# struan-robertson/shoeprint-image-retrieval

Measured on AMD Instinct MI355X. Metric: query x gallery NCC pairs/sec, higher is better.
Workload: dtype f32; 1 GPU; config 2: WVU2019-shaped VGG16 conv3_3 NCC: Q=100 x G=1500 (1500/GPU), features [256,128,64] stored as float32, rotations/scales none, queries signal 1 / noise 126; method=fft, gallery_chunk=1500, storage=float32, parallelism=gallery-shard x1, streams=1

## Files before the change

shoeprint-image-retrieval_amd/csrc/ncc_fft.hip:

```cpp
#include <cstdlib>

#include "fft_core.h"
#include "ncc_fft_cfg.h"
#include "ncc_prep_common.h"

#ifndef SPR_BIG_ABL
#define SPR_BIG_ABL 0
#endif
namespace spr {
namespace {

inline int rt_stride(int r_rows) { return r_rows + ((8 - r_rows % 32) + 32) % 32; }

template <class C, bool BIG, int PT>
__global__ void __launch_bounds__(PT)
prep_fft_kernel(NccGeom g, int is_query, const void* __restrict__ maps, unsigned char* __restrict__ prepared,
                size_t item_bytes, const cf* __restrict__ tw_h, const cf* __restrict__ tw_w, unsigned x0_off,
                unsigned f_off, unsigned xbuf_off, unsigned zbuf_off, unsigned sat2_off, int f_stride,
                unsigned char* __restrict__ ws, size_t slot_bytes) {
  using GH = typename C::GH;
  using GW = typename C::GW;
  unsigned char* lds = dyn_lds();
  unsigned char* big = lds;
  if constexpr (BIG) big = ws + (static_cast<size_t>(blockIdx.y) * gridDim.x + blockIdx.x) * slot_bytes;
// ... 516 lines not shown
#pragma unroll
          for (int s = 0; s < KW; ++s) {
            const cf v = y[pp][s];
            const int e = (pp * KW + s) * 2;
            const int n2 = GW::out_index(tr, pp, s);
            const int n1 = 2 * (rr * C::PPR + gr);
            const bool ok = GW::out_valid(tr, pp) && n2 < g.iw;
            if (ok && n1 < g.ih) maps_out[(static_cast<size_t>(c) * g.ih + n1) * g.iw + n2] = v.x * ivf[e];
            if (ok && n1 + 1 < g.ih) maps_out[(static_cast<size_t>(c) * g.ih + n1 + 1) * g.iw + n2] = v.y * ivf[e + 1];
          }
        }
      }
    }
    store_nyq();
    __syncthreads();
  }

  float best = 0.0f;
#pragma unroll
  for (int r = 0; r < RR; ++r)
#pragma unroll
    for (int e = 0; e < NV; ++e) best = fmaxf(best, acc[r][e]);
  best = block_max<C::NT>(best, red);
  if (tid == 0 && scores) {
    const float s = best / static_cast<float>(g.channels);
    float* dst = scores + static_cast<size_t>(qi) * ld + col0 + gi_item;
    const float prev = g.accumulate ? *dst : 0.0f;
    *dst = s > prev ? s : prev;
  }
  }
}

struct PrepFftLds {
  size_t x0_off, f_off, xbuf_off, zbuf_off, sat2_off, total;
  int f_stride;
  size_t slot_bytes;
};
template <class C>
PrepFftLds prep_fft_lds(const NccGeom& g, bool is_query, int pt) {
  const int h = is_query ? g.th : g.ih, w = is_query ? g.tw : g.iw;
  PrepFftLds l;
  l.f_stride = C::NW / 2 + 1;
  const size_t f_bytes = sizeof(cf) * static_cast<size_t>(2 * ((h + 1) / 2)) * l.f_stride;
  const size_t sat_bytes = align_up(sizeof(double) * (h + 1) * (w + 1), 16);
  if (g.big) {
    l.xbuf_off = 64;
    l.zbuf_off = l.xbuf_off;
    l.total = l.xbuf_off + sizeof(cf) * C::prep_xbuf_elems(pt);
    l.x0_off = 0;
    l.f_off = align_up(sizeof(float) * h * w, 256);
    const size_t first = f_bytes > sat_bytes ? f_bytes : sat_bytes;
    l.sat2_off = align_up(l.f_off + first, 256);
    l.slot_bytes = align_up(l.sat2_off + (is_query ? 0 : sat_bytes), 256);
    return l;
  }
  l.slot_bytes = 0;
  l.x0_off = 64;
  l.f_off = align_up(l.x0_off + sizeof(float) * h * w, 16);
  l.xbuf_off = align_up(l.f_off + f_bytes, 16);
  l.zbuf_off = l.xbuf_off;
  const size_t fft_total = l.xbuf_off + sizeof(cf) * C::prep_xbuf_elems(pt);
  size_t sat_total = is_query ? 0 : l.f_off + sat_bytes;
  l.sat2_off = 0;
  if (!is_query && l.f_off + 2 * sat_bytes <= static_cast<size_t>(kLdsLimit)) {
    l.sat2_off = l.f_off + sat_bytes;
    sat_total = l.f_off + 2 * sat_bytes;
  }
  l.total = fft_total > sat_total ? fft_total : sat_total;
  return l;
}

struct PairFftLds {
  size_t r_off, xbuf_off, nyq_off, total, slot_bytes;
};
template <class C>
constexpr int rk_tuned() { return C::RR_A * C::PPR * 2 < C::NH ? C::RR_A * C::PPR * 2 : C::NH; }

template <class C>
PairFftLds pair_fft_lds(const NccGeom& g) {
  PairFftLds l;
  l.r_off = 64;
  const size_t r_bytes = sizeof(cf) * static_cast<size_t>(C::COLS) * g.r_stride;
  l.slot_bytes = g.big ? align_up(r_bytes, 256) : 0;
  l.xbuf_off = align_up(l.r_off + (g.big ? 0 : r_bytes), 16);
  l.nyq_off = align_up(l.xbuf_off + sizeof(cf) * C::xbuf_elems(C::NT), 16);
  l.total = l.nyq_off + sizeof(cf) * (2 * C::NH + C::NH + C::NW);
  return l;
}

struct FftEntry {
  int nh, nw, eh, tgh, ew, tgw, nt, spl_w;
  int kw_a, rr_a, kw_b, rr_b, rk_a;
  bool pow2;
  int spec_per_chan;
  size_t (*prep_lds_total)(const NccGeom&, bool);
  size_t (*pair_lds_total)(const NccGeom&);
  int (*prep)(const NccGeom&, const PlanScratch&, const PrepCall&);
  int (*pair)(const NccGeom&, const PlanScratch&, const PairCall&);
  size_t (*prep_slot_bytes)(const NccGeom&, bool);
  size_t (*pair_slot_bytes)(const NccGeom&);
  bool big_only;
  bool six;
};

template <class C>
int prep_threads(const NccGeom& g, bool q) {
  if (C::NH * C::NW >= 128 * 64 && prep_fft_lds<C>(g, q, 512).total <= static_cast<size_t>(kLdsLimit)) return 512;
  return kThreads;
}
template <class C>
size_t prep_lds_total_t(const NccGeom& g, bool q) { return prep_fft_lds<C>(g, q, prep_threads<C>(g, q)).total; }
template <class C>
size_t pair_lds_total_t(const NccGeom& g) { return pair_fft_lds<C>(g).total; }
template <class C>
size_t prep_slot_bytes_t(const NccGeom& g, bool q) { return prep_fft_lds<C>(g, q, kThreads).slot_bytes; }
template <class C>
size_t pair_slot_bytes_t(const NccGeom& g) { return pair_fft_lds<C>(g).slot_bytes; }

template <class C, bool BIG, int PT>
int prep_launch(const NccGeom& g, const PlanScratch& s, const PrepCall& c) {
  const PrepFftLds l = prep_fft_lds<C>(g, c.is_query, PT);
  const size_t item_bytes = c.is_query ? prepared_query_item_bytes(g, SPR_NCC_FFT) : prepared_gallery_item_bytes(g, SPR_NCC_FFT);
  (void)hipFuncSetAttribute(reinterpret_cast<const void*>(prep_fft_kernel<C, BIG, PT>),
                            hipFuncAttributeMaxDynamicSharedMemorySize, kLdsLimit);
  int64_t batch = c.n;
  if (BIG) {
    const size_t per_item = l.slot_bytes * static_cast<size_t>(g.channels);
    if (!s.ws || s.ws_bytes < per_item) { set_error("prep_fft_kernel: workspace too small for one item"); return SPR_ERR_WORKSPACE; }
    batch = static_cast<int64_t>(s.ws_bytes / per_item);
  }
  const int raw_h = c.is_query ? g.q_h : g.g_h, raw_w = c.is_query ? g.q_w : g.g_w;
  const size_t elem = g.dtype == SPR_F32 ? 4 : 2;
  const size_t raw_item_bytes = static_cast<size_t>(g.channels) * raw_h * raw_w * elem;
  for (int64_t first = 0; first < c.n; first += batch) {
    const int64_t m = c.n - first < batch ? c.n - first : batch;
    hipLaunchKernelGGL(HIP_KERNEL_NAME(prep_fft_kernel<C, BIG, PT>), dim3(g.channels, static_cast<unsigned>(m)), dim3(PT),
                       l.total, c.stream, g, c.is_query ? 1 : 0,
                       static_cast<const void*>(static_cast<const unsigned char*>(c.maps) + first * raw_item_bytes),
                       static_cast<unsigned char*>(c.prepared) + first * item_bytes, item_bytes, s.tw_h,
                       s.tw_w, static_cast<unsigned>(l.x0_off), static_cast<unsigned>(l.f_off),
                       static_cast<unsigned>(l.xbuf_off), static_cast<unsigned>(l.zbuf_off),
                       static_cast<unsigned>(l.sat2_off), l.f_stride, static_cast<unsigned char*>(s.ws), l.slot_bytes);
    const int rc = check_launch("prep_fft_kernel");
    if (rc != SPR_OK) return rc;
  }
  return SPR_OK;
}
template <class C>
int prep_t(const NccGeom& g, const PlanScratch& s, const PrepCall& c) {
#ifndef SPR_SAN_SUBSET
  if (g.big) return prep_launch<C, true, kThreads>(g, s, c);
#endif
  if (prep_threads<C>(g, c.is_query) == 512) return prep_launch<C, false, 512>(g, s, c);
  return prep_launch<C, false, kThreads>(g, s, c);
}

constexpr int kTeamCounters = 8 * 32;

template <class C, int RR, int KW, int PF, int RK, bool BIG, bool TEAM>
int pair_launch(const NccGeom& g, const PlanScratch& s, const PairCall& c) {
  const int64_t nq = c.nq, ng = c.ng;
  unsigned* team_sync = c.maps_out && !BIG ? nullptr : s.team_sync;
  const PairFftLds l = pair_fft_lds<C>(g);
  const int64_t tiles = static_cast<int64_t>(ceil_div(static_cast<int>(nq), kTileQ)) * ceil_div(static_cast<int>(ng), kTileG);
  PairArgs a{};
  a.channels = g.channels; a.nq = static_cast<int>(nq); a.ng = static_cast<int>(ng);
  a.ih = g.ih; a.iw = g.iw; a.r_rows = g.r_rows; a.r_stride = g.r_stride; a.rounds_r = g.rounds_r;
  a.inv_per_chan = g.inv_per_chan; a.accumulate = c.accumulate;
  const void* kernel = reinterpret_cast<const void*>(pair_fft_kernel<C, RR, KW, PF, RK, BIG, TEAM>);
  (void)hipFuncSetAttribute(kernel, hipFuncAttributeMaxDynamicSharedMemorySize, kLdsLimit);
  unsigned grid = 0;
  int per_cu = 0, cus = 0, dev = 0;
  if (TEAM && !team_sync) { set_error("pair_fft_kernel: the team schedule needs the plan's counters"); return SPR_ERR_ARG; }
  if (TEAM && hipGetDevice(&dev) == hipSuccess &&
      hipDeviceGetAttribute(&cus, hipDeviceAttributeMultiprocessorCount, dev) == hipSuccess &&
      hipOccupancyMaxActiveBlocksPerMultiprocessor(&per_cu, pair_fft_kernel<C, RR, KW, PF, RK, BIG, TEAM>, C::NT, l.total) == hipSuccess &&
      per_cu > 0 && cus >= 8) {
    int team_size = cus / 8 * per_cu;
    if (BIG) {
      const size_t slots = s.ws ? s.ws_bytes / l.slot_bytes : 0;
      if (slots < 8) { set_error("pair_fft_kernel: workspace too small"); return SPR_ERR_WORKSPACE; }
      if (static_cast<size_t>(team_size) * 8 > slots) team_size = static_cast<int>(slots / 8);
    }
    {
      const int strip_max = env_int("SPR_NCC_STRIP_Q", 16) > 0 ? env_int("SPR_NCC_STRIP_Q", 16) : 16;
      const int strips = ceil_div(static_cast<int>(nq), strip_max);
      a.team_size = team_size;
      a.strips = strips;
      a.strip_q = ceil_div(static_cast<int>(nq), strips);
      a.strips = ceil_div(static_cast<int>(nq), a.strip_q);
      a.epochs_full = static_cast<int>((static_cast<int64_t>(a.strip_q) * ng + team_size - 1) / team_size);
      const int q_last = static_cast<int>(nq) - (a.strips - 1) * a.strip_q;
      a.epochs_total = (a.strips - 1) * a.epochs_full + static_cast<int>((static_cast<int64_t>(q_last) * ng + team_size - 1) / team_size);
      a.sync_polls = env_int("SPR_NCC_TEAM_POLLS", BIG ? 0 : 256);
      a.sync_every = env_int("SPR_NCC_TEAM_EVERY", BIG ? 0 : 32);
      if (a.sync_every < 0) a.sync_every = 0;
      grid = 8u * static_cast<unsigned>(team_size);
      if (hipMemsetAsync(team_sync, 0, sizeof(unsigned) * kTeamCounters, c.stream) != hipSuccess) {
        set_error("hipMemsetAsync(team counters) failed");
        return SPR_ERR_HIP;
      }
    }
  }
  if (TEAM && a.team_size == 0) { set_error("pair_fft_kernel: could not size the persistent grid"); return SPR_ERR_HIP; }
  const int64_t max_tiles = TEAM ? tiles : pair_tiles_per_launch(kTileQ * kTileG, C::NT);
  for (int64_t t0 = 0; t0 < (TEAM ? 1 : tiles); t0 += max_tiles) {
    if (!TEAM) {
      const int64_t n = tiles - t0 < max_tiles ? tiles - t0 : max_tiles;
      a.tile0 = static_cast<int>(t0);
      grid = static_cast<unsigned>(n * kTileQ * kTileG);
    }
    hipLaunchKernelGGL(HIP_KERNEL_NAME(pair_fft_kernel<C, RR, KW, PF, RK, BIG, TEAM>), dim3(grid),
                       dim3(C::NT), l.total, c.stream, a, static_cast<const unsigned char*>(c.pq),
                       prepared_query_item_bytes(g, SPR_NCC_FFT), static_cast<const unsigned char*>(c.pg),
                       prepared_gallery_item_bytes(g, SPR_NCC_FFT), c.scores,
                       static_cast<long long>(c.ld), static_cast<long long>(c.col0), c.maps_out, s.tw_h, s.tw_w,
                       static_cast<unsigned>(l.r_off), static_cast<unsigned>(l.xbuf_off),
                       static_cast<unsigned>(l.nyq_off), team_sync, static_cast<unsigned char*>(s.ws), l.slot_bytes);
    const int rc = check_launch("pair_fft_kernel");
    if (rc != SPR_OK) return rc;
  }
  (void)kernel;
  return SPR_OK;
}

constexpr int kBigMidKw = 11, kBigMidRr = 4;
template <class C, int PFA, bool BIG, bool TEAM>
int pair_tb(const NccGeom& g, const PlanScratch& s, const PairCall& c) {
  if (g.tight) return pair_launch<C, C::RR_A, C::KW_A, PFA, rk_tuned<C>(), BIG, TEAM>(g, s, c);
  if constexpr (BIG) {
    if (g.keep_w == kBigMidKw) return pair_launch<C, kBigMidRr, kBigMidKw, 1, 0, BIG, TEAM>(g, s, c);
  }
  return pair_launch<C, C::RR_B, C::KW_B, 1, 0, BIG, TEAM>(g, s, c);
}
template <class C, int PFA>
int pair_t(const NccGeom& g, const PlanScratch& s, const PairCall& c) {
#ifndef SPR_SAN_SUBSET
  if (g.big) return pair_tb<C, PFA, true, true>(g, s, c);
  if (s.team_sync && !c.maps_out && team_schedule()) return pair_tb<C, PFA, false, true>(g, s, c);
#endif
  return pair_tb<C, PFA, false, false>(g, s, c);
}

template <class C, int PFA, bool BIG_ONLY = false>
constexpr FftEntry entry() {
  return FftEntry{C::NH,   C::NW,   C::EH,   C::TGH,  C::EW,   C::TGW, C::NT, C::GW::SPL,
                  C::KW_A, C::RR_A, C::KW_B, C::RR_B, rk_tuned<C>(),
                  (C::NH & (C::NH - 1)) == 0 && (C::NW & (C::NW - 1)) == 0,
                  C::kSpecPerChan, prep_lds_total_t<C>, pair_lds_total_t<C>, prep_t<C>, pair_t<C, PFA>,
                  prep_slot_bytes_t<C>, pair_slot_bytes_t<C>, BIG_ONLY, false};
}

size_t pair6_lds_total(const NccGeom&) { return pair6_lds_bytes(); }
size_t no_slot_bytes(const NccGeom&) { return 0; }
template <class C>
constexpr FftEntry entry6() {
  return FftEntry{C::NH, C::NW, C::EH, C::TGH, C::EW, C::TGW, C::NT, C::GW::SPL, 0, 0, 0, 0, 0, false,
                  C::kSpecPerChan, prep_lds_total_t<C>, pair6_lds_total, prep_t<C>, launch_pair6,
                  prep_slot_bytes_t<C>, no_slot_bytes, false, true};
}

#ifdef SPR_SAN_SUBSET
const FftEntry kEntries[] = {
    entry<Cfg<8, 4, 4, 4, 64, 2, 1>, 1>(),
    entry<Cfg<12, 8, 6, 8, 192, 5, 2>, 1>(),
    entry6<Cfg<12, 16, 12, 8, 384, 5, 2, 1>>(),
    entry<Cfg<12, 16, 12, 8, 256, 5, 2>, 1>(),
};
#else
const FftEntry kEntries[] = {
    entry<Cfg<8, 4, 4, 4, 64, 2, 1>, 1>(),
    entry<Cfg<8, 4, 8, 4, 64, 2, 1>, 1>(),
    entry<Cfg<12, 4, 6, 4, 64, 2, 1>, 1>(),
    entry<Cfg<8, 8, 8, 4, 64, 2, 1>, 1>(),
    entry<Cfg<8, 8, 8, 8, 256, 4, 1>, 1>(),
    entry<Cfg<12, 8, 6, 8, 192, 5, 2>, 1>(),
    entry<Cfg<16, 8, 8, 8, 256, 4, 1>, 1>(),
    entry<Cfg<16, 8, 16, 8, 256, 4, 1>, 1>(),
    entry6<Cfg<12, 16, 12, 8, 384, 5, 2, 1>>(),
    entry<Cfg<12, 16, 12, 8, 256, 5, 2>, 1>(),
    entry<Cfg<16, 16, 16, 8, 512, 4, 1>, 2>(),
    entry<Cfg<24, 16, 12, 16, 512, 9, 4>, 1, true>(),
};
#endif

const FftEntry* find_entry(int nh, int nw, int six) {
  for (const FftEntry& e : kEntries)
    if (e.nh == nh && e.nw == nw && (e.six ? 1 : 0) == six) return &e;
  return nullptr;
}

inline int fft_need(int img, int tpl) {
  const int c = tpl / 2;
  const int a = img + c, b = img + tpl - 1 - c;
  return a > b ? a : b;
}

bool fill_geometry(NccGeom& g, const FftEntry& e, bool big) {
  g.big = big ? 1 : 0;
  g.six = e.six ? 1 : 0;
  g.nh = e.nh; g.nw = e.nw; g.eh = e.eh; g.tgh = e.tgh; g.ew = e.ew; g.tgw = e.tgw; g.nt = e.nt;
  if (e.six) {
    if (big || env_int("SPR_NCC_SIX", 1) == 0) return false;
    if (g.ih > pair6_max_rows() || g.iw > pair6_max_cols()) return false;
    g.rounds_c = 2; g.r_rows = g.ih; g.r_stride = 0; g.rounds_r = 1; g.tight = 1; g.keep_w = 0; g.nv = 24;
    g.spec_per_chan = e.spec_per_chan;
    g.inv_per_chan = 6 * e.nt * 4;
    if (g.ih * g.iw > kMaxPixPerThread * kThreads || g.th * g.tw > kMaxPixPerThread * kThreads) return false;
    if (e.prep_lds_total(g, true) > static_cast<size_t>(kLdsLimit)) return false;
    if (e.prep_lds_total(g, false) > static_cast<size_t>(kLdsLimit)) return false;
    return e.pair_lds_total(g) <= static_cast<size_t>(kLdsLimit);
  }
  const int cpr = e.nt / e.tgh, ppr = e.nt / e.tgw;
  g.rounds_c = ceil_div(e.nw / 2, cpr);
  g.r_rows = (g.ih + 7) / 8 * 8;
  if (g.r_rows > e.nh) g.r_rows = e.nh;
  g.rounds_r = ceil_div(g.r_rows / 2, ppr);
  const int kw_need = ceil_div(g.iw, e.ew);
  const bool tuned = kw_need <= e.kw_a && g.rounds_r <= e.rr_a;
  g.r_stride = rt_stride(tuned ? e.rk_a : g.r_rows);
  g.tight = tuned ? 1 : 0;
  g.keep_w = tuned ? e.kw_a : e.kw_b;
  if (!tuned && (kw_need > e.kw_b || g.rounds_r > e.rr_b)) return false;
  if (big && !tuned && kw_need <= kBigMidKw && g.rounds_r <= kBigMidRr && kBigMidKw < e.kw_b) g.keep_w = kBigMidKw;
  g.nv = (e.spl_w * g.keep_w * 2 + 3) / 4 * 4;
  g.spec_per_chan = e.spec_per_chan;
  g.inv_per_chan = g.rounds_r * g.nv * e.nt;
  if (!big && (g.ih * g.iw > kMaxPixPerThread * kThreads || g.th * g.tw > kMaxPixPerThread * kThreads)) return false;
  if (e.prep_lds_total(g, true) > static_cast<size_t>(kLdsLimit)) return false;
  if (e.prep_lds_total(g, false) > static_cast<size_t>(kLdsLimit)) return false;
  if (e.pair_lds_total(g) > static_cast<size_t>(kLdsLimit)) return false;
  return true;
}

}

bool fft_geometry(NccGeom& g, bool pow2_only) {
  const int need_h = fft_need(g.ih, g.th), need_w = fft_need(g.iw, g.tw);
  const int min_h = need_h > g.th ? need_h : g.th, min_w = need_w > g.tw ? need_w : g.tw;
  const FftEntry* best = nullptr;
  NccGeom best_g = g;
  const bool force_big = env_int("SPR_NCC_FORCE_BIG", 0) == 1;
#ifdef SPR_SAN_SUBSET
  constexpr int kPasses = 1;
#else
  constexpr int kPasses = 2;
#endif
  for (int pass = force_big ? 1 : 0; pass < kPasses && !best; ++pass) {
    for (const FftEntry& e : kEntries) {
      if (e.nh < min_h || e.nw < min_w) continue;
      if (pow2_only && !e.pow2) continue;
      if (pass == 0 && e.big_only) continue;
      if (best && static_cast<long long>(e.nh) * e.nw >= static_cast<long long>(best->nh) * best->nw) continue;
      NccGeom trial = g;
      if (!fill_geometry(trial, e, pass == 1)) continue;
      best = &e;
      best_g = trial;
    }
  }
  if (!best) return false;
  g = best_g;
  return true;
}

size_t fft_workspace_bytes(const NccGeom& g) {
  if (!g.big) return 0;
  const FftEntry* e = find_entry(g.nh, g.nw, g.six);
  if (!e) return 0;
  const size_t prep_q = e->prep_slot_bytes(g, true), prep_g = e->prep_slot_bytes(g, false);
  const size_t prep = (prep_q > prep_g ? prep_q : prep_g) * static_cast<size_t>(g.channels) * 2;
  const size_t pair = e->pair_slot_bytes(g) * 512;
  return prep > pair ? prep : pair;
}

int launch_prep_fft(const NccGeom& g, const PlanScratch& s, const PrepCall& c) {
  if (c.n == 0) return SPR_OK;
  const FftEntry* e = find_entry(g.nh, g.nw, g.six);
  if (!e) { set_error("no FFT kernel for grid %dx%d", g.nh, g.nw); return SPR_ERR_UNSUPPORTED; }
  return e->prep(g, s, c);
}

int launch_pair_fft(const NccGeom& g, const PlanScratch& s, const PairCall& c) {
  if (c.nq == 0 || c.ng == 0) return SPR_OK;
  const FftEntry* e = find_entry(g.nh, g.nw, g.six);
  if (!e) { set_error("no FFT kernel for grid %dx%d", g.nh, g.nw); return SPR_ERR_UNSUPPORTED; }
  return e->pair(g, s, c);
}

#ifdef SPR_PREP_STAMPS
extern "C" int spr_debug_read_prep_stamps(unsigned long long* host, int n) {
  return hipMemcpyFromSymbol(host, HIP_SYMBOL(g_prep_stamps), sizeof(unsigned long long) * n) == hipSuccess ? 0 : -1;
}
#endif

}
```

shoeprint-image-retrieval_amd/csrc/spr_common.h:

```cpp
#pragma once
#include <hip/hip_runtime.h>
#include <stddef.h>
#include <stdint.h>

#include "../../include/shoeprint_mi355x.h"
#include <spr_intrinsics.h>

namespace spr {

constexpr int kThreads = 256;
constexpr int kLdsLimit = 160 * 1024;

typedef float cf __attribute__((ext_vector_type(2)));
static_assert(sizeof(cf) == 8, "cf must be 8 bytes");

__host__ __device__ inline int ceil_div(int a, int b) { return (a + b - 1) / b; }
__host__ __device__ inline size_t align_up(size_t v, size_t a) { return (v + a - 1) / a * a; }

void set_error(const char* fmt, ...);
int check_launch(const char* what);

struct NccGeom {
  int channels;
  int q_h, q_w, g_h, g_w;
  int crop;
  int th, tw, ih, iw;
  int dtype;
  int nh, nw;
  int nt;
  int eh, tgh, ew, tgw;
  int big;
  int six;
  int tight;
  int rounds_c;
  int r_rows;
  int r_stride;
  int rounds_r;
  int keep_w;
  int nv;
  int spec_per_chan;
  int inv_per_chan;
  int pad_h, pad_w;
  int strips_per_row;
  int strips_per_thread;
  int mfma_exact;
  int mfma_general;
  int mfma_f32;
};

constexpr int kStrip = 8;

struct PairCall {
  const void* pq; int64_t nq;
  const void* pg; int64_t ng;
  float* scores; int64_t ld, col0; int accumulate;
  float* maps_out;
  hipStream_t stream;
};
struct PrepCall {
  bool is_query;
  const void* maps; int64_t n;
  void* prepared;
  hipStream_t stream;
};
struct PlanScratch {
  cf* tw_h; cf* tw_w;
  unsigned* team_sync;
  void* ws; size_t ws_bytes;
  float* six_ctab;
  float* mfma_x;
};

int env_int(const char* name, int fallback);
bool team_schedule();

int launch_prep_direct(const NccGeom& g, const PlanScratch& s, const PrepCall& c);
int launch_pair_direct(const NccGeom& g, const PlanScratch& s, const PairCall& c);
int launch_prep_fft(const NccGeom& g, const PlanScratch& s, const PrepCall& c);
int launch_pair_fft(const NccGeom& g, const PlanScratch& s, const PairCall& c);
int launch_pair6(const NccGeom& g, const PlanScratch& s, const PairCall& c);
int launch_prep_mfma(const NccGeom& g, const PlanScratch& s, const PrepCall& c);
int launch_pair_mfma(const NccGeom& g, const PlanScratch& s, const PairCall& c);
int64_t pair_tiles_per_launch(int pairs_per_tile, int threads);

size_t pair6_lds_bytes();
int pair6_max_rows();
int pair6_max_cols();
size_t fft_workspace_bytes(const NccGeom& g);
bool mfma_geometry(NccGeom& g);
bool mfma_f32_geometry(NccGeom& g);
size_t mfma_query_item_bytes(const NccGeom& g);
size_t mfma_gallery_item_bytes(const NccGeom& g);
size_t mfma_workspace_bytes(const NccGeom& g);
bool fft_geometry(NccGeom& g, bool pow2_only);
bool direct_geometry(NccGeom& g);

size_t prepared_query_item_bytes(const NccGeom& g, int method);
size_t prepared_gallery_item_bytes(const NccGeom& g, int method);

__device__ __forceinline__ float load_feature(const void* base, size_t idx, int dtype) {
  if (dtype == SPR_F32) return static_cast<const float*>(base)[idx];
  const uint16_t bits = static_cast<const uint16_t*>(base)[idx];
  if (dtype == SPR_BF16) {
    union { uint32_t u; float f; } v;
    v.u = static_cast<uint32_t>(bits) << 16;
    return v.f;
  }
  union { uint16_t u; _Float16 h; } v;
  v.u = bits;
  return static_cast<float>(v.h);
}

__host__ __device__ inline uint16_t round_bf16(float v) {
  union { float f; uint32_t u; } c;
  c.f = v;
  if ((c.u & 0x7fffffffu) > 0x7f800000u) return 0x7fc0;
  c.u += 0x7fffu + ((c.u >> 16) & 1u);
  return static_cast<uint16_t>(c.u >> 16);
}
__device__ __forceinline__ uint16_t round_f16(float v) {
  union { _Float16 h; uint16_t u; } c;
  c.h = static_cast<_Float16>(v);
  return c.u;
}
template <int KIND>
__device__ __forceinline__ uint16_t round16(float v) { return KIND == SPR_F16 ? round_f16(v) : round_bf16(v); }
template <int KIND>
__device__ __forceinline__ float value16(uint16_t b) {
  if (KIND == SPR_F16) {
    union { uint16_t u; _Float16 h; } c;
    c.u = b;
    return static_cast<float>(c.h);
  }
  union { uint32_t u; float f; } c;
  c.u = static_cast<uint32_t>(b) << 16;
  return c.f;
}

__device__ __forceinline__ double block_sum(double v, double* scratch) {
  for (int m = 32; m >= 1; m >>= 1) v += shfl_xor(v, m);
  const int tid = static_cast<int>(threadIdx.x);
  __syncthreads();
  if ((tid & 63) == 0) scratch[tid >> 6] = v;
  __syncthreads();
  double s = 0.0;
  for (int w = 0; w < static_cast<int>(blockDim.x) / 64; ++w) s += scratch[w];
  return s;
}
template <int NT = kThreads>
__device__ __forceinline__ float block_max(float v, float* scratch) {
  for (int m = 32; m >= 1; m >>= 1) v = fmaxf(v, shfl_xor(v, m));
  const int tid = static_cast<int>(threadIdx.x);
  __syncthreads();
  if ((tid & 63) == 0) scratch[tid >> 6] = v;
  __syncthreads();
  float s = scratch[0];
  for (int w = 1; w < NT / 64; ++w) s = fmaxf(s, scratch[w]);
  return s;
}

}
```

Baseline: 275,700 pairs/s.

## Add dedicated gallery prep kernel for six-step FFT path processing multiple channels per workgroup

Adds a new gallery preparation kernel for the six-step FFT geometry. Each 512-thread workgroup handles 8 channels, prefetching the next channel's features into registers while the current one is processed. Within a channel it computes mean and energy, builds integral images with segmented parallel prefix sums, writes the inverse-sigma tables, and runs row and column FFTs in LDS. The aim is to cut gallery prep cost, which counts toward pairs/s. The price is a large, complex new code path that carries correctness risk.

```diff
diff --git a/shoeprint-image-retrieval_amd/csrc/ncc_fft.hip b/shoeprint-image-retrieval_amd/csrc/ncc_fft.hip
--- a/shoeprint-image-retrieval_amd/csrc/ncc_fft.hip
+++ b/shoeprint-image-retrieval_amd/csrc/ncc_fft.hip
@@ -842,6 +842,7 @@
   g.nh = e.nh; g.nw = e.nw; g.eh = e.eh; g.tgh = e.tgh; g.ew = e.ew; g.tgw = e.tgw; g.nt = e.nt;
   if (e.six) {
     if (big || env_int("SPR_NCC_SIX", 1) == 0) return false;
+    g.prep6 = env_int("SPR_PREP6", 1) != 0 ? 1 : 0;
     if (g.ih > pair6_max_rows() || g.iw > pair6_max_cols()) return false;
     g.rounds_c = 2; g.r_rows = g.ih; g.r_stride = 0; g.rounds_r = 1; g.tight = 1; g.keep_w = 0; g.nv = 24;
     g.spec_per_chan = e.spec_per_chan;
@@ -917,6 +918,7 @@
   if (c.n == 0) return SPR_OK;
   const FftEntry* e = find_entry(g.nh, g.nw, g.six);
   if (!e) { set_error("no FFT kernel for grid %dx%d", g.nh, g.nw); return SPR_ERR_UNSUPPORTED; }
+  if (!c.is_query && prep6_covers(g)) return launch_prep6(g, s, c);
   return e->prep(g, s, c);
 }
 
diff --git a/shoeprint-image-retrieval_amd/csrc/ncc_prep6.hip b/shoeprint-image-retrieval_amd/csrc/ncc_prep6.hip
--- /dev/null
+++ b/shoeprint-image-retrieval_amd/csrc/ncc_prep6.hip
@@ -0,0 +1,366 @@
+#include "fft_core.h"
+#include "ncc_fft_cfg.h"
+#include "ncc_prep_common.h"
+
+namespace spr {
+namespace {
+
+using C6 = Cfg<12, 16, 12, 8, 384, 5, 2, 1>;
+constexpr int kPT = 512;
+constexpr int kLoads = 16;
+constexpr int kSeg = 4;
+constexpr int kRowSeg = 16;
+constexpr int kChansPerWg = 8;
+
+#ifdef SPR_PREP6_STAMPS
+__device__ unsigned long long g_prep6_stamps[16];
+#define SPR_PSTAMP6(i) do { if (blockIdx.x == 12 && blockIdx.y == 700 && c == c_first + 1 && threadIdx.x == 0) g_prep6_stamps[i] = __builtin_amdgcn_s_memtime(); } while (0)
+#else
+#define SPR_PSTAMP6(i)
+#endif
+
+struct Prep6Lds {
+  size_t x0_off, f_off, xbuf_off, tw_off, total;
+  int f_stride;
+};
+Prep6Lds prep6_lds(const NccGeom& g) {
+  const int h = g.ih, w = g.iw;
+  Prep6Lds l;
+  l.f_stride = C6::NW / 2 + 1;
+  const size_t f_bytes = sizeof(cf) * static_cast<size_t>(2 * ((h + 1) / 2)) * l.f_stride;
+  l.x0_off = 64;
+  l.f_off = align_up(l.x0_off + sizeof(float) * h * w, 16);
+  l.xbuf_off = align_up(l.f_off + f_bytes, 16);
+  const size_t fft_total = l.xbuf_off + sizeof(cf) * C6::prep_xbuf_elems(kPT);
+  const size_t stat_total = l.f_off + 2 * sizeof(double) * static_cast<size_t>(h) * w;
+  l.tw_off = align_up(fft_total > stat_total ? fft_total : stat_total, 16);
+  l.total = l.tw_off + sizeof(cf) * (C6::NW + C6::NH);
+  return l;
+}
+
+__device__ __forceinline__ void stretch_offsets(double t, int sg, int d, double& off, double& tot) {
+  const double a = shfl_xor(t, d), b = shfl_xor(t, 2 * d), c = shfl_xor(t, 3 * d);
+  off = 0.0;
+  tot = 0.0;
+#pragma unroll
+  for (int j = 0; j < kSeg; ++j) {
+    const double v = j == sg ? t : (j == (sg ^ 1) ? a : (j == (sg ^ 2) ? b : c));
+    off += j < sg ? v : 0.0;
+    tot += v;
+  }
+}
+
+__global__ void __launch_bounds__(kPT)
+prep6_gallery_kernel(NccGeom g, const void* __restrict__ maps, unsigned char* __restrict__ prepared, size_t item_bytes,
+                     const cf* __restrict__ tw_h, const cf* __restrict__ tw_w, unsigned x0_off, unsigned f_off,
+                     unsigned xbuf_off, unsigned tw_off, int f_stride) {
+  using C = C6;
+  using GH = typename C::GH;
+  using GW = typename C::GW;
+  unsigned char* lds = dyn_lds();
+  double* red = reinterpret_cast<double*>(lds);
+  float* x0 = reinterpret_cast<float*>(lds + x0_off);
+  cf* F = reinterpret_cast<cf*>(lds + f_off);
+  cf* xbuf = reinterpret_cast<cf*>(lds + xbuf_off);
+  const int tid = static_cast<int>(threadIdx.x);
+  const size_t item = blockIdx.y;
+  const int h = g.ih, w = g.iw, n = h * w;
+  double* H1 = reinterpret_cast<double*>(lds + f_off);
+  double* H2 = H1 + n;
+  const int c_first = static_cast<int>(blockIdx.x) * kChansPerWg;
+  const int c_end = c_first + kChansPerWg < g.channels ? c_first + kChansPerWg : g.channels;
+
+  unsigned char* item_base = prepared + item * item_bytes;
+  const size_t spec_bytes = sizeof(cf) * static_cast<size_t>(g.channels) * C::kSpecPerChan;
+  unsigned char* flags = item_base + spec_bytes + sizeof(float) * static_cast<size_t>(g.channels) * g.inv_per_chan;
+
+  const int dy = kPT / w, dx = kPT - dy * w;
+  const int y_first = tid / w, x_first = tid - y_first * w;
+  float v[kLoads];
+  auto request = [&](int c) {
+    const size_t chan_base = (item * g.channels + c) * static_cast<size_t>(g.g_h) * g.g_w;
+    int yy = y_first, xx = x_first;
+#pragma unroll
+    for (int k = 0; k < kLoads; ++k) {
+      v[k] = tid + k * kPT < n
+                 ? load_feature(maps, chan_base + static_cast<size_t>(yy + g.crop) * g.g_w + (xx + g.crop), g.dtype)
+                 : 0.0f;
+      xx += dx; yy += dy;
+      if (xx >= w) { xx -= w; ++yy; }
+    }
+  };
+  request(c_first);
+
+  cf* twt_w = reinterpret_cast<cf*>(lds + tw_off);
+  cf* twt_h = twt_w + C::NW;
+  for (int k = tid; k < C::NW; k += kPT) twt_w[k] = tw_w[(k / C::TGW) * (k % C::TGW)];
+  for (int k = tid; k < C::NH; k += kPT) twt_h[k] = tw_h[(k / C::TGH) * (k % C::TGH)];
+
+  const int cy = g.th / 2, cx = g.tw / 2;
+  const int above = g.th - cy, left = g.tw - cx;
+  const double inv_n = 1.0 / (static_cast<double>(g.th) * static_cast<double>(g.tw));
+
+  for (int c = c_first; c < c_end; ++c) {
+    SPR_PSTAMP6(0);
+    double s = 0.0;
+#pragma unroll
+    for (int k = 0; k < kLoads; ++k)
+      if (tid + k * kPT < n) s += static_cast<double>(v[k]);
+    const double total = block_sum(s, red);
+    const float mean = static_cast<float>(total / static_cast<double>(n));
+    double e = 0.0;
+#pragma unroll
+    for (int k = 0; k < kLoads; ++k) {
+      if (tid + k * kPT < n) {
+        const float d = v[k] - mean;
+        x0[tid + k * kPT] = d;
+        const float sq = d * d;
+        e += static_cast<double>(sq);
+      }
+    }
+    SPR_PSTAMP6(1);
+    const float energy = static_cast<float>(block_sum(e, red));
+    const float rs = energy > 0.0f ? static_cast<float>(1.0 / sqrt(static_cast<double>(energy))) : 0.0f;
+    if (tid == 0) flags[c] = rs == 0.0f ? 1 : 0;
+    if (c + 1 < c_end) request(c + 1);
+    SPR_PSTAMP6(2);
+
+    {
+      const int tidv = opaque(tid);
+      const int u = tidv < h * kSeg ? tidv : h * kSeg - 1;
+      const bool live = tidv < h * kSeg;
+      const int y = u / kSeg, sg = u - y * kSeg;
+      const int wseg = (w + kSeg - 1) / kSeg;
+      const int xa = sg * wseg < w ? sg * wseg : w;
+      const int cnt = w - xa < wseg ? w - xa : wseg;
+      const float* src = x0 + y * w;
+      float tv[kRowSeg];
+#pragma unroll
+      for (int k = 0; k < kRowSeg; ++k) {
+        const float t = src[xa + k < w ? xa + k : w - 1];
+        tv[k] = k < cnt ? t : 0.0f;
+      }
+      double r1 = 0.0, r2 = 0.0;
+#pragma unroll
+      for (int k = 0; k < kRowSeg; ++k) {
+        const float sq = tv[k] * tv[k];
+        r1 += static_cast<double>(tv[k]);
+        r2 += static_cast<double>(sq);
+      }
+      double q1, q2, t1, t2;
+      stretch_offsets(r1, sg, 1, q1, t1);
+      stretch_offsets(r2, sg, 1, q2, t2);
+      double* h1 = H1 + y * w;
+      double* h2 = H2 + y * w;
+      if (live) {
+#pragma unroll
+        for (int k = 0; k < kRowSeg; ++k) {
+          const float sq = tv[k] * tv[k];
+          q1 += static_cast<double>(tv[k]);
+          q2 += static_cast<double>(sq);
+          const int kk = xa + k + 1;
+          if (k < cnt && kk < w) {
+            const int xl = kk - left;
+            if (xl >= 0 && xl <= cx) { h1[xl] = q1; h2[xl] = q2; }
+            const int xr = kk + cx;
+            if (xr < w) { h1[xr] = t1 - q1; h2[xr] = t2 - q2; }
+          }
+        }
+        if (cnt > 0 && xa + cnt == w) {
+          int xl = w - left < 0 ? 0 : w - left;
+          const int xe = cx < w - 1 ? cx : w - 1;
+          for (; xl <= xe; ++xl) { h1[xl] = q1; h2[xl] = q2; }
+        }
+      }
+    }
+    __syncthreads();
+    SPR_PSTAMP6(7);
+
+    {
+      const int tidv = opaque(tid);
+      const int xcol = ((tidv >> 6) & 3) * 16 + (tidv & 15), csg = (tidv >> 4) & 3;
+      const int hseg = (h + kSeg - 1) / kSeg;
+      const int ya = csg * hseg < h ? csg * hseg : h;
+      const int ycnt = xcol < w ? (h - ya < hseg ? h - ya : hseg) : 0;
+      double* col = ((tidv >> 8) ? H2 : H1) + ya * w + (xcol < w ? xcol : w - 1);
+      constexpr int B = 8;
+      double r = 0.0;
+      for (int k0 = 0; k0 < ycnt; k0 += B) {
+        double t[B];
+#pragma unroll
+        for (int k = 0; k < B; ++k) t[k] = col[(k0 + k < ycnt ? k0 + k : ycnt - 1) * w];
+#pragma unroll
+        for (int k = 0; k < B; ++k) r += k0 + k < ycnt ? t[k] : 0.0;
+      }
+      double run, tot;
+      stretch_offsets(r, csg, 16, run, tot);
+      for (int k0 = 0; k0 < ycnt; k0 += B) {
+        double t[B];
+#pragma unroll
+        for (int k = 0; k < B; ++k) t[k] = col[(k0 + k < ycnt ? k0 + k : ycnt - 1) * w];
+#pragma unroll
+        for (int k = 0; k < B; ++k) {
+          run += k0 + k < ycnt ? t[k] : 0.0;
+          col[(k0 + k < ycnt ? k0 + k : ycnt - 1) * w] = run;
+        }
+      }
+    }
+    __syncthreads();
+    SPR_PSTAMP6(8);
+    {
+      float4* inv4 = reinterpret_cast<float4*>(item_base + spec_bytes) + static_cast<size_t>(c) * (g.inv_per_chan / 4);
+      for (int idx4 = opaque(tid); idx4 < C::kInv6PerChan / 4; idx4 += kPT) {
+        const int pp = idx4 / C::NT, lane6 = idx4 - pp * C::NT;
+        const int l64 = lane6 & 63, rg = l64 / 3, tq = l64 - 3 * rg;
+        const int row = (lane6 >> 6) * C::kRowGroups + rg, n1 = 3 * pp + tq;
+        float o[4] = {0.0f, 0.0f, 0.0f, 0.0f};
+        if (l64 < 63 && n1 < 16 && row < h) {
+          const int b = (33 * n1) % 48;
+          const int ma = tq == 1 ? b - 32 : b, mb = ma == n1 ? n1 + 16 : n1;
+          const bool upper = row <= cy;
+          const int hi = upper ? (row + above < h ? row + above : h) - 1 : h - 1;
+          const int lo = upper ? 0 : row - cy - 1;
+          const double* p1a = H1 + hi * w;
+          const double* p1b = H1 + lo * w;
+          const double* p2a = H2 + hi * w;
+          const double* p2b = H2 + lo * w;
+          double a1[4], b1[4], a2[4], b2[4];
+#pragma unroll
+          for (int e = 0; e < 4; ++e) {
+            const int x = 2 * (e < 2 ? ma : mb) + (e & 1), xs = x < w ? x : w - 1;
+            a1[e] = p1a[xs]; b1[e] = p1b[xs]; a2[e] = p2a[xs]; b2[e] = p2b[xs];
+          }
+#pragma unroll
+          for (int e = 0; e < 4; ++e) {
+            const int x = 2 * (e < 2 ? ma : mb) + (e & 1);
+            const float r = inv_sigma_from_sums(upper ? a1[e] : a1[e] - b1[e], upper ? a2[e] : a2[e] - b2[e], inv_n);
+            o[e] = x < w ? r : 0.0f;
+          }
+        }
+        inv4[idx4] = float4{o[0], o[1], o[2], o[3]};
+      }
+    }
+    __syncthreads();
+    SPR_PSTAMP6(3);
+
+    {
+      const int tidv = opaque(tid);
+      const int giw = tidv / C::TGW, t = tidv - giw * C::TGW;
+      const LdsTwiddles<C::TGW> twr{twt_w, t};
+      cf* gbuf = xbuf + giw * C::kRowGroupElems;
+      cf* zb = gbuf;
+      const int pairs = (h + 1) / 2;
+      constexpr int kPairsPerRound = kPT / C::TGW;
+      const int rounds = ceil_div(pairs, kPairsPerRound);
+      for (int rr = 0; rr < rounds; ++rr) {
+        const int pr = rr * kPairsPerRound + giw;
+        const int ra = 2 * pr, rb = ra + 1;
+        cf x[C::EW], y[GW::SPL][C::TGW];
+#pragma unroll
+        for (int m = 0; m < C::EW; ++m) {
+          const int n2 = GW::in_index(t, m);
+          const bool in = n2 < w;
+          x[m].x = (in && ra < h) ? x0[ra * w + n2] : 0.0f;
+          x[m].y = (in && rb < h) ? x0[rb * w + n2] : 0.0f;
+        }
+        group_fft<C::EW, C::TGW, -1>(x, y, t, twr, gbuf);
+        wave_sync();
+#pragma unroll
+        for (int pp = 0; pp < GW::SPL; ++pp)
+#pragma unroll
+          for (int sidx = 0; sidx < C::TGW; ++sidx)
+            if (GW::out_valid(t, pp)) zb[GW::out_index(t, pp, sidx)] = y[pp][sidx];
+        wave_sync();
+        if (pr < pairs) {
+          for (int k = t; k <= C::NW / 2; k += C::TGW) {
+            const cf zk = zb[k];
+            const cf zm = zb[k == 0 ? 0 : C::NW - k];
+            F[ra * f_stride + k] = cmake(0.5f * (zk.x + zm.x), 0.5f * (zk.y - zm.y));
+            F[rb * f_stride + k] = cmake(0.5f * (zk.y + zm.y), 0.5f * (zm.x - zk.x));
+          }
+        }
+        wave_sync();
+      }
+    }
+    __syncthreads();
+    SPR_PSTAMP6(4);
+
+    {
+      cf* spec = reinterpret_cast<cf*>(item_base) + static_cast<size_t>(c) * C::kSpecPerChan;
+      const int tidv = opaque(tid);
+      const int gi = tidv / C::TGH, t = tidv - gi * C::TGH;
+      const LdsTwiddles<C::TGH> twc{twt_h, t};
+      cf* gbuf = xbuf + gi * GH::kGroupElems;
+      const int rows_f = 2 * ((h + 1) / 2);
+      constexpr int kColsPerRound = kPT / C::TGH;
+      constexpr int kRounds = (C::COLS + 1 + kColsPerRound - 1) / kColsPerRound;
+      for (int rc = 0; rc < kRounds; ++rc) {
+        const int j = rc * kColsPerRound + gi;
+        const bool nyq = j == C::COLS;
+        const bool active = j <= C::COLS;
+        cf x[C::EH], y[GH::SPL][C::TGH];
+#pragma unroll
+        for (int m = 0; m < C::EH; ++m) {
+          const int n1 = GH::in_index(t, m);
+          x[m] = (active && n1 < rows_f) ? F[n1 * f_stride + j] : cmake(0.0f, 0.0f);
+        }
+        group_fft<C::EH, C::TGH, -1>(x, y, t, twc, gbuf);
+        if (active) {
+#pragma unroll
+          for (int pp = 0; pp < GH::SPL; ++pp) {
+            if (!GH::out_valid(t, pp)) continue;
+#pragma unroll
+            for (int sidx = 0; sidx < C::TGH; ++sidx) {
+              const int k1 = GH::out_index(t, pp, sidx);
+              spec[nyq ? C::kNyqOffset + k1 : C::spec_index(C::slot(j), k1)] = y[pp][sidx];
+            }
+          }
+        }
+      }
+    }
+    __syncthreads();
+    SPR_PSTAMP6(5);
+  }
+}
+
+}
+
+bool prep6_covers(const NccGeom& g) {
+  if (!g.six || g.big || !g.prep6) return false;
+  if (g.nh != C6::NH || g.nw != C6::NW || g.nt != C6::NT) return false;
+  if (g.th < g.ih || g.tw < g.iw) return false;
+  if (g.ih > C6::kRows6 || g.ih * kSeg > kPT || g.iw > 64) return false;
+  if (g.ih * g.iw > kLoads * kPT) return false;
+  if (g.inv_per_chan != C6::kInv6PerChan) return false;
+  return prep6_lds(g).total <= static_cast<size_t>(kLdsLimit);
+}
+
+int launch_prep6(const NccGeom& g, const PlanScratch& s, const PrepCall& c) {
+  const Prep6Lds l = prep6_lds(g);
+  const size_t item_bytes = prepared_gallery_item_bytes(g, SPR_NCC_FFT);
+  (void)hipFuncSetAttribute(reinterpret_cast<const void*>(prep6_gallery_kernel),
+                            hipFuncAttributeMaxDynamicSharedMemorySize, kLdsLimit);
+  const size_t elem = g.dtype == SPR_F32 ? 4 : 2;
+  const size_t raw_item_bytes = static_cast<size_t>(g.channels) * g.g_h * g.g_w * elem;
+  const int64_t batch = 65535;
+  for (int64_t first = 0; first < c.n; first += batch) {
+    const int64_t m = c.n - first < batch ? c.n - first : batch;
+    hipLaunchKernelGGL(prep6_gallery_kernel, dim3(ceil_div(g.channels, kChansPerWg), static_cast<unsigned>(m)), dim3(kPT),
+                       l.total, c.stream, g,
+                       static_cast<const void*>(static_cast<const unsigned char*>(c.maps) + first * raw_item_bytes),
+                       static_cast<unsigned char*>(c.prepared) + first * item_bytes, item_bytes, s.tw_h, s.tw_w,
+                       static_cast<unsigned>(l.x0_off), static_cast<unsigned>(l.f_off), static_cast<unsigned>(l.xbuf_off),
+                       static_cast<unsigned>(l.tw_off), l.f_stride);
+    const int rc = check_launch("prep6_gallery_kernel");
+    if (rc != SPR_OK) return rc;
+  }
+  return SPR_OK;
+}
+
+#ifdef SPR_PREP6_STAMPS
+extern "C" int spr_debug_read_prep_stamps(unsigned long long* host, int n) {
+  return hipMemcpyFromSymbol(host, HIP_SYMBOL(g_prep6_stamps), sizeof(unsigned long long) * n) == hipSuccess ? 0 : -1;
+}
+#endif
+
+}
diff --git a/shoeprint-image-retrieval_amd/csrc/spr_common.h b/shoeprint-image-retrieval_amd/csrc/spr_common.h
--- a/shoeprint-image-retrieval_amd/csrc/spr_common.h
+++ b/shoeprint-image-retrieval_amd/csrc/spr_common.h
@@ -31,6 +31,7 @@
   int eh, tgh, ew, tgw;
   int big;
   int six;
+  int prep6;
   int tight;
   int rounds_c;
   int r_rows;
@@ -79,6 +80,8 @@
 int launch_prep_fft(const NccGeom& g, const PlanScratch& s, const PrepCall& c);
 int launch_pair_fft(const NccGeom& g, const PlanScratch& s, const PairCall& c);
 int launch_pair6(const NccGeom& g, const PlanScratch& s, const PairCall& c);
+bool prep6_covers(const NccGeom& g);
+int launch_prep6(const NccGeom& g, const PlanScratch& s, const PrepCall& c);
 int launch_prep_mfma(const NccGeom& g, const PlanScratch& s, const PrepCall& c);
 int launch_pair_mfma(const NccGeom& g, const PlanScratch& s, const PairCall& c);
 int64_t pair_tiles_per_launch(int pairs_per_tile, int threads);
```

Result: faster. 279,000 pairs/s, median of 6 (+1.2%).
